# dbolya/yolact

Measured on AMD Instinct MI355X. Metric: images/sec (550x550, batch 8 per GPU), YOLACT yolact_resnet50 forward + Detect (Fast NMS), higher is better.
Workload: dtype f32 (fp32 in / fp32 accumulate / fp32 out; 93 % of the GEMM time on fp16x2 tiles = every fp32 operand as two fp16 pieces by round to nearest (22 significant bits + 2 signs: exact for ~2/3 of all fp32 values, one fp32 ulp otherwise), 3 exact piece products per product on the fp16 matrix pipe; measure

## Files before the change

### yolact_amd/csrc/common.h

```cpp
#pragma once
#include <hip/hip_runtime.h>
#include <stdint.h>

#define YMI_OK 0
#define YMI_EARG (-1)
#define YMI_ESHAPE (-2)
#define YMI_ENULL (-3)

typedef float f32x4 __attribute__((ext_vector_type(4)));
typedef float f32x16 __attribute__((ext_vector_type(16)));

static inline int ymi_launch_status() {
  hipError_t e = hipGetLastError();
  return e == hipSuccess ? YMI_OK : (int)e;
}

__device__ __forceinline__ int ymi_lane() { return threadIdx.x & 63; }

__device__ __forceinline__ int ymi_xcd_remap(int bid, int nwg) {
  const int q = nwg >> 3, r = nwg & 7, xcd = bid & 7, local = bid >> 3;
  const int base = (xcd < r) ? xcd * (q + 1) : r * (q + 1) + (xcd - r) * q;
  return base + local;
}

__host__ __device__ __forceinline__ void ymi_h2_scale(float amax, float &s, float &inv) {
  const unsigned u = __builtin_bit_cast(unsigned, amax);
  const int eb = (int)((u >> 23) & 0xff);
  int es = 267 - eb;
  if (eb == 0 || eb == 255) es = 127;
  es = es < 2 ? 2 : (es > 252 ? 252 : es);
  s = __builtin_bit_cast(float, (unsigned)es << 23);
  inv = __builtin_bit_cast(float, (unsigned)(254 - es) << 23);
}

#define YMI_AMAX_SUB 16
#define YMI_AMAX_STRIDE 64
struct ymi_amax_pre { float *sub; unsigned cur; };
__device__ __forceinline__ unsigned ymi_wave_umax63(unsigned v) {
  auto step = [](unsigned x, unsigned y) { return x > y ? x : y; };
  v = step(v, (unsigned)__builtin_amdgcn_update_dpp(0, (int)v, 0xb1, 0xf, 0xf, false));
  v = step(v, (unsigned)__builtin_amdgcn_update_dpp(0, (int)v, 0x4e, 0xf, 0xf, false));
  v = step(v, (unsigned)__builtin_amdgcn_update_dpp(0, (int)v, 0x114, 0xf, 0xf, false));
  v = step(v, (unsigned)__builtin_amdgcn_update_dpp(0, (int)v, 0x118, 0xf, 0xf, false));
  v = step(v, (unsigned)__builtin_amdgcn_update_dpp(0, (int)v, 0x142, 0xa, 0xf, false));
  v = step(v, (unsigned)__builtin_amdgcn_update_dpp(0, (int)v, 0x143, 0xc, 0xf, false));
  return v;
}
__device__ __forceinline__ ymi_amax_pre ymi_amax_prefetch(float *slot) {
  ymi_amax_pre p;
  const unsigned xcc = (unsigned)__builtin_amdgcn_s_getreg((3 << 11) | (0 << 6) | 20) & 7u;
  p.sub = slot ? slot + (2 * xcc + ((blockIdx.x + blockIdx.y) & 1)) * YMI_AMAX_STRIDE : nullptr;
  p.cur = 0xffffffffu;
  if (slot && (threadIdx.x & 63) == 63)
    p.cur = __hip_atomic_load(reinterpret_cast<const unsigned *>(p.sub), __ATOMIC_RELAXED, __HIP_MEMORY_SCOPE_WORKGROUP);
  return p;
}
// ... 27 lines not shown
```

### yolact_amd/csrc/conv_igemm.hip

```cpp
#include "common.h"
#include <stdlib.h>
#include <mutex>
#include <type_traits>
#include "../../include/yolact_amd.h"

namespace {

constexpr int BK = 32;
constexpr unsigned OOB = 0x80000000u;

typedef __attribute__((address_space(3))) void *lds_ptr_t;
typedef unsigned u32x4 __attribute__((ext_vector_type(4)));
typedef __bf16 bf16x8 __attribute__((ext_vector_type(8)));

struct Split3 { bf16x8 h, m, l; };

__device__ __forceinline__ Split3 split8(const f32x4 x0, const f32x4 x1) {
  const float x[8] = {x0[0], x0[1], x0[2], x0[3], x1[0], x1[1], x1[2], x1[3]};
  unsigned r1[8], r2[8];
#pragma unroll
  for (int e = 0; e < 8; ++e) {
    const float h = __builtin_bit_cast(float, __builtin_bit_cast(unsigned, x[e]) & 0xFFFF0000u);
    const float r = x[e] - h;
    r1[e] = __builtin_bit_cast(unsigned, r);
// ... 2 lines not shown
  }
  u32x4 ph, pm, pl;
#pragma unroll
  for (int q = 0; q < 4; ++q) {
    ph[q] = __builtin_amdgcn_perm(__builtin_bit_cast(unsigned, x[2 * q + 1]), __builtin_bit_cast(unsigned, x[2 * q]), 0x07060302u);
    pm[q] = __builtin_amdgcn_perm(r1[2 * q + 1], r1[2 * q], 0x07060302u);
    pl[q] = __builtin_amdgcn_perm(r2[2 * q + 1], r2[2 * q], 0x07060302u);
  }
  Split3 s;
  s.h = __builtin_bit_cast(bf16x8, ph); s.m = __builtin_bit_cast(bf16x8, pm); s.l = __builtin_bit_cast(bf16x8, pl);
  return s;
}


typedef _Float16 f16x8 __attribute__((ext_vector_type(8)));
struct Split2 { f16x8 h, l; };

__device__ __forceinline__ Split2 split8h(const f32x4 x0, const f32x4 x1, const float s) {
  const float x[8] = {x0[0], x0[1], x0[2], x0[3], x1[0], x1[1], x1[2], x1[3]};
  Split2 o;
#pragma unroll
  for (int e = 0; e < 8; ++e) {
    const float t = x[e] * s;
    const _Float16 h = (_Float16)t;
    o.h[e] = h;
    o.l[e] = (_Float16)(t - (float)h);
  }
  return o;
}

struct KParams {
  ymi_conv_desc d;
  int M, HoWo, tiles_n, nk;
  unsigned x_bytes, w_bytes;
  const float *offmask;
  int ldo, mask_is_prob, om_layout;
  long x_gs, w_gs, y_gs;
  const void *w3;
  unsigned w3_plane;
  unsigned w3_gs;
  const void *a2;
  unsigned a2_plane;
  long a2_gs;
  unsigned sc_gs;
  unsigned long long *trace;
  int abl;
};

__device__ __forceinline__ float act_apply(float v, int act) {
  switch (act) {
    case YMI_ACT_RELU: return v > 0.f ? v : 0.f;
    case YMI_ACT_LEAKY01: return v > 0.f ? v : 0.1f * v;
    case YMI_ACT_TANH: return tanhf(v);
    case YMI_ACT_SIGMOID: return 1.f / (1.f + expf(-v));
    default: return v;
  }
}

__device__ __forceinline__ void bilin_coord(int dst, float scale, int in_size, int &i0, int &i1, float &l1) {
  float src = scale * ((float)dst + 0.5f) - 0.5f;
  src = src < 0.f ? 0.f : src;
  i0 = (int)src;
  if (i0 > in_size - 1) i0 = in_size - 1;
  i1 = i0 + ((i0 < in_size - 1) ? 1 : 0);
  l1 = src - (float)i0;
}
// ... 118 lines not shown
  constexpr int NWAVE = WM * WN * WK, NTHR = 64 * NWAVE;
  constexpr int RPP = NTHR / 8;
  constexpr int NPL = (PREC == 2) ? 3 : 2;
  constexpr bool BPL = PREC >= 2;
  constexpr bool APL = PREC == 4;
  constexpr bool H2 = PREC >= 3;
  constexpr int RA = APL ? (2 * BM) / (16 * NWAVE) : BM / RPP, RB = BPL ? (NPL * BN) / (16 * NWAVE) : BN / RPP;
  static_assert((APL ? (2 * BM) % (16 * NWAVE) == 0 : BM % RPP == 0) && (BPL ? (NPL * BN) % (16 * NWAVE) == 0 : BN % RPP == 0),
                "tile rows must be a multiple of the rows per staging pass");
  static_assert(!APL || LOADER == 3, "pre-split A planes: pointwise loader only");
  constexpr int SUB = conv_sub_floats<BM, BN, PREC>();
  constexpr int STAGE = SUB * WK;
  constexpr int NS = (LOADER == 2) ? 2 : NSTAGE;
  constexpr int DMA_PER_STEP = (RA + RB) * WK;
  constexpr int ELD = BN + 4;
  constexpr int LDS_FLOATS = (NS * STAGE > WK * BM * ELD) ? NS * STAGE : WK * BM * ELD;
  static_assert(DMA_PER_STEP * (NS - 2) <= 63, "vmcnt is a 6-bit counter");
  static_assert(WM * WN * WK == 4 || WM * WN * WK == 8, "4 or 8 waves per block");
  static_assert(LOADER != 2 || WK == 1, "DCN gather runs without the K split");
  static_assert(PREC == 0 || PREC == 3 || LOADER != 2, "the DCN gather: exact-fp32 or fp16x2 (A split on the fly from the fp32 LDS image)");
  static_assert(!BPL || BN % 16 == 0, "16-bit planes: 16-row DMA pieces");
  __shared__ __attribute__((aligned(16))) float lds[LDS_FLOATS];

  const ymi_conv_desc &d = p.d;
  const int t = threadIdx.x;
  const int lane = t & 63, wave = __builtin_amdgcn_readfirstlane(t >> 6);
  const int wk = wave % WK, wmn = wave / WK;
  const int wm = wmn / WN, wn = wmn % WN;
  const int kq = t & 7, r0 = t >> 3;
  const int sl = kq ^ ((r0 >> 1) & 7);

  unsigned long long tr_t0 = 0, tr_loop = 0, tr_epi = 0, tr_tp = 0, tr_c = 0;
  if (p.trace) tr_t0 = __builtin_readcyclecounter();
  const int logical = ymi_xcd_remap(blockIdx.x, gridDim.x);
  const int tile_n = logical % p.tiles_n, tile_m = logical / p.tiles_n;
  const int m0 = tile_m * BM, n0 = tile_n * BN;

  const int grp = blockIdx.y;
  const __amdgpu_buffer_rsrc_t xrs = APL
      ? __builtin_amdgcn_make_buffer_rsrc((void *)((const char *)p.a2 + (size_t)grp * p.a2_gs), 0, (int)(2 * p.a2_plane), 0x00020000)
      : __builtin_amdgcn_make_buffer_rsrc((void *)(d.x + (size_t)grp * p.x_gs), 0, (int)p.x_bytes, 0x00020000);
  const __amdgpu_buffer_rsrc_t wrs = BPL
      ? __builtin_amdgcn_make_buffer_rsrc((void *)((const char *)p.w3 + (size_t)grp * p.w3_gs), 0, (int)(NPL * p.w3_plane), 0x00020000)
      : __builtin_amdgcn_make_buffer_rsrc((void *)(d.w + (size_t)grp * p.w_gs), 0, (int)p.w_bytes, 0x00020000);
  float sA = 1.f, invA = 1.f;
  if (H2) {
    float xam = d.x_amax ? ymi_amax_read(d.x_amax) : 0.f;
    if (d.x_amax_mul != 0.f) xam *= d.x_amax_mul;
    ymi_h2_scale(xam, sA, invA);
  }
  const ymi_amax_pre apre = ymi_amax_prefetch(d.y_amax);

  constexpr int C4 = BN / 4;
  constexpr int RSTEP = NTHR / C4;
  constexpr int RPT = BM / RSTEP;
  constexpr bool RES_PREFETCH = RPT <= 8;
  const int c4 = t % C4, rbase = t / C4;
  const int n = n0 + 4 * c4;
  const bool vec_res = (d.res_ld & 3) == 0 && ((((uintptr_t)d.res) & 15) == 0) && (n + 3 < d.Cout);
  f32x4 rpre[RES_PREFETCH ? RPT : 1];
  if (RES_PREFETCH && d.res_mode == YMI_RES_ADD && vec_res) {
#pragma unroll
    for (int i = 0; i < RPT; ++i) {
      const int m = m0 + rbase + RSTEP * i;
      const f32x4 z = {0.f, 0.f, 0.f, 0.f};
      rpre[i] = (m < p.M) ? *reinterpret_cast<const f32x4 *>(d.res + (size_t)m * d.res_ld + n) : z;
    }
  }

  const float *scp = H2 ? d.scale_h2 + (size_t)grp * p.sc_gs : d.scale;
  f32x4 sc = {1.f, 1.f, 1.f, 1.f}, bi = {0.f, 0.f, 0.f, 0.f};
// ... 594 lines not shown
      epilogue_general<BM, BN, WK, RPT, RSTEP, RES_PREFETCH>(p, es, sc, bi, rpre, m0, n, c4, rbase, vec_res, invA, apre);
    }
  }
  if (p.trace && t == 0) {
    const unsigned hw = __builtin_amdgcn_s_getreg((31 << 11) | (0 << 6) | 4);
    const unsigned xcc = __builtin_amdgcn_s_getreg((3 << 11) | (0 << 6) | 20);
    unsigned long long *o = p.trace + (size_t)blockIdx.x * 8;
    o[0] = ((unsigned long long)xcc << 32) | hw;
    o[1] = tr_t0; o[2] = tr_loop; o[3] = tr_epi; o[4] = __builtin_readcyclecounter(); o[5] = tr_tp; o[6] = tr_c;
  }
#endif
}

struct ProfRec { hipEvent_t e0, e1; double flops; int tile; int kind; };
constexpr int PROF_MAX = 4096;
ProfRec g_prof[PROF_MAX];
unsigned long long *g_trace = nullptr;
long g_trace_cap = 0;
int g_prof_n = 0, g_prof_alloc = 0, g_prof_on = 0;
std::mutex g_prof_mu;

constexpr int LDS_PER_CU = 160 * 1024, NUM_CU = 256;

template <int WM, int WN, int WK, int TM, int TN, int NS, bool ALL_LOADERS, int PREC>
int launch_cfg(const KParams &kp, int loader, hipStream_t s, int groups) {
  constexpr int BM = WM * TM * 32, BN = WN * TN * 32;
  constexpr int ns_eff_bytes = NS * conv_sub_floats<BM, BN, PREC>() * WK * 4, epi_bytes = WK * BM * (BN + 4) * 4;
  constexpr int static_lds = ns_eff_bytes > epi_bytes ? ns_eff_bytes : epi_bytes;
  KParams p = kp;
  const int tiles_m = (p.M + BM - 1) / BM;
  p.tiles_n = (p.d.Cout + BN - 1) / BN;
  const int grid = tiles_m * p.tiles_n;
  if (p.trace && (grid > g_trace_cap || groups > 1)) p.trace = nullptr;
  int dyn = 0;
  {
    int occ = LDS_PER_CU / static_lds;
    if (PREC >= 1) {
      constexpr int occ_regs = conv_occupancy<WM, WN, WK, TM, TN, NS, 0, PREC>();
      occ = occ < occ_regs ? occ : occ_regs;
    }
    const int k = (grid * groups + NUM_CU - 1) / NUM_CU;
    if (k < occ && !(p.abl & 8)) {
      const int want = LDS_PER_CU / (k + 1) + 1024;
      if (want > static_lds && want <= LDS_PER_CU / k) dyn = want - static_lds;
    }
  }
  const bool pointwise = p.d.kh == 1 && p.d.kw == 1 && p.d.pad == 0;
  if constexpr (PREC == 4) {
    if (loader != 0 || !pointwise) return YMI_EARG;
    hipLaunchKernelGGL((conv_igemm_f32<WM, WN, WK, TM, TN, NS, 3, 4>), dim3(grid, groups), dim3(64 * WM * WN * WK), dyn, s, p);
    return ymi_launch_status();
  } else
  if (loader == 0 && (groups > 1 || pointwise)) {
    hipLaunchKernelGGL((conv_igemm_f32<WM, WN, WK, TM, TN, NS, 3, PREC>), dim3(grid, groups), dim3(64 * WM * WN * WK), dyn, s, p);
  } else if (loader == 0) {
    hipLaunchKernelGGL((conv_igemm_f32<WM, WN, WK, TM, TN, NS, 0, PREC>), dim3(grid, groups), dim3(64 * WM * WN * WK), dyn, s, p);
  } else if constexpr (ALL_LOADERS) {
    if (loader == 1) hipLaunchKernelGGL((conv_igemm_f32<WM, WN, WK, TM, TN, NS, 1, PREC>), dim3(grid, groups), dim3(64 * WM * WN * WK), dyn, s, p);
    else if constexpr (PREC == 0) hipLaunchKernelGGL((conv_igemm_f32<WM, WN, WK, TM, TN, NS, 2, 0>), dim3(grid, groups), dim3(64 * WM * WN * WK), dyn, s, p);
    else if constexpr (PREC == 3) hipLaunchKernelGGL((conv_igemm_f32<WM, WN, WK, TM, TN, NS, 2, 3>), dim3(grid, groups), dim3(64 * WM * WN * WK), dyn, s, p);
    else return YMI_EARG;
  } else {
    return YMI_EARG;
  }
  return ymi_launch_status();
}
// ... 402 lines not shown
```

### yolact_amd/csrc/dcn.hip

```cpp
#include "common.h"
#include <stdlib.h>
#include <type_traits>
#include "../../include/yolact_amd.h"

int ymi_internal_prof_begin(double flops, int tile, int kind, hipStream_t s);
void ymi_internal_prof_end(int idx, hipStream_t s);

#ifndef YMI_A_AUX
#define YMI_A_AUX 0
#endif

namespace {

constexpr int BK = 32;
constexpr unsigned OOB = 0x80000000u;

typedef __attribute__((address_space(3))) void *lds_ptr_t;
typedef unsigned u32x4 __attribute__((ext_vector_type(4)));
typedef unsigned u32x3 __attribute__((ext_vector_type(3)));
typedef _Float16 f16x8 __attribute__((ext_vector_type(8)));
typedef _Float16 f16x4 __attribute__((ext_vector_type(4)));
struct Split2 { f16x8 h, l; };

struct DcnParams {
  const float *x, *offmask, *scale_h2, *bias, *x_amax;
  const void *w_h2;
  float *y, *y_amax;
  int B, H, W, Cin, ldx, Ho, Wo, Cout, stride, Kpad, ldo, ldy, act, mask_is_prob;
  int taps, kw, pad;
  const float *res; int res_ld, res_after_act;
  int M, HoWo, tiles_n, nk;
  int nk_split;
  long y_gs;
  unsigned x_bytes, om_bytes, w_plane;
  int om_layout;
  int abl;
  unsigned long long *trace;
  int trace_mode;
};

template <int WM, int WN, int TM, int TN, int RING>
constexpr int dcn_lds_floats() {
  constexpr int BM = WM * TM * 32, BN = WN * TN * 32;
  constexpr int pipe = 2 * (2 * BM * 16) + (RING + 2) * (2 * BN * 16), epi = BM * (BN + 4);
  return pipe > epi ? pipe : epi;
}
template <int WM, int WN, int TM, int TN, int RING, bool PLAIN>
constexpr int dcn_occupancy() {
  constexpr int occ = (160 * 1024) / (dcn_lds_floats<WM, WN, TM, TN, RING>() * 4);
  constexpr int nw = WM * WN, ra = (WM * TM * 32) / (8 * nw);
  constexpr int cap = (!PLAIN && (nw > 8 || (nw == 8 && ra > 1))) ? 1 : (WN * TN == 1 && nw <= 4) ? 4 : 2;
  return occ > cap ? cap : (occ < 1 ? 1 : occ);
}

template <int WM, int WN, int TM, int TN, int RING, bool PLAIN>
__global__ __launch_bounds__(64 * WM * WN, (dcn_occupancy<WM, WN, TM, TN, RING, PLAIN>() * (WM * WN) + 3) / 4)
void pipe_h2_k(const DcnParams p) {
#if defined(__HIP_DEVICE_COMPILE__)
  constexpr int BM = WM * TM * 32, BN = WN * TN * 32, NW = WM * WN, NT = 64 * NW;
  constexpr int RPP = NT / 8, RA = BM / RPP;
  constexpr int BUNITS = (2 * BN) / 16;
  constexpr int RB = (BUNITS + NW - 1) / NW;
  static_assert(BM % RPP == 0 && RA >= 1, "tile rows vs gather passes");
  static_assert(RING == 1 || RING == 2, "ring depth");
  constexpr int NSB = RING + 2;
  constexpr int A_STAGE = 2 * BM * 16, B_STAGE = 2 * BN * 16;
  constexpr int NC = PLAIN ? 1 : 4;
  constexpr int NG = NC * RA, NB = RB;
  constexpr int N_STEADY = RING * (NG + NB);
  static_assert(N_STEADY <= 63, "vmcnt is a 6-bit counter");
  constexpr int ELD = BN + 4;
  constexpr int LDS_FLOATS = dcn_lds_floats<WM, WN, TM, TN, RING>();
  __shared__ __attribute__((aligned(16))) float lds[LDS_FLOATS];
  float *const Abase = lds, *const Bbase = lds + 2 * A_STAGE;

  const int t = threadIdx.x;
  const int lane = t & 63, wave = __builtin_amdgcn_readfirstlane(t >> 6);
  const int wm = wave / WN, wn = wave % WN;
  const int kq = t & 7, r0 = t >> 3;
#ifdef YMI_DIAGNOSTICS
  unsigned long long tr_[10] = {0, 0, 0, 0, 0, 0, 0, 0, 0, 0}, tr_rt0 = 0;
  const bool tracing = p.trace != nullptr;
#define YMI_STAMP(i) do { if (tracing) tr_[i] = __builtin_amdgcn_s_memtime(); } while (0)
  if (tracing) tr_rt0 = __builtin_amdgcn_s_memrealtime();
  YMI_STAMP(0);
#else
#define YMI_STAMP(i) do { } while (0)
#endif

  const int logical = ymi_xcd_remap(blockIdx.x, gridDim.x);
  const int tile_n = logical % p.tiles_n, tile_m = logical / p.tiles_n;
  const int m0 = tile_m * BM, n0 = tile_n * BN;

  const __amdgpu_buffer_rsrc_t xrs = __builtin_amdgcn_make_buffer_rsrc((void *)p.x, 0, (int)p.x_bytes, 0x00020000);
  const __amdgpu_buffer_rsrc_t ors = __builtin_amdgcn_make_buffer_rsrc((void *)p.offmask, 0, (int)p.om_bytes, 0x00020000);
  const __amdgpu_buffer_rsrc_t wrs = __builtin_amdgcn_make_buffer_rsrc((void *)p.w_h2, 0, (int)(2 * p.w_plane), 0x00020000);

  float sA, invA;
  ymi_h2_scale(ymi_amax_read(p.x_amax), sA, invA);
  const ymi_amax_pre apre = ymi_amax_prefetch(p.y_amax);
#ifdef YMI_DIAGNOSTICS
  if (tracing && p.trace_mode == 2) {
    unsigned long long tt;
    asm volatile("s_memtime %0\n\ts_waitcnt lgkmcnt(0)" : "=s"(tt) : "s"(__builtin_amdgcn_readfirstlane(__builtin_bit_cast(int, sA))) : "memory");
    tr_[1] = tt;
  }
#endif

  constexpr int C4 = BN / 4, RSTEP = NT / C4, RPT = BM / RSTEP;
  const int c4 = t % C4, rbase = t / C4;
  const int n = n0 + 4 * c4;
  int g_iy0[RA], g_ix0[RA], g_ib[RA];
  unsigned g_om[RA];
  int a_st[RA];
#pragma unroll
  for (int i = 0; i < RA; ++i) {
    const int row = r0 + RPP * i, m = m0 + row;
    a_st[i] = row * 64 + (((kq >> 1) ^ ((row >> 2) & 3)) * 16) + (kq & 1) * 8;
    if (m < p.M) {
      const int b = m / p.HoWo, pix = m - b * p.HoWo;
      const int oy = pix / p.Wo, ox = pix - oy * p.Wo;
      g_iy0[i] = oy * p.stride - (PLAIN ? p.pad : 1);
      g_ix0[i] = ox * p.stride - (PLAIN ? p.pad : 1);
      g_ib[i] = b * p.H * p.W;
// ... 345 lines not shown
      o[10] = tr_rt0;
      o[11] = __builtin_amdgcn_s_memrealtime();
      o[12] = (unsigned long long)__builtin_amdgcn_s_getreg((31 << 11) | (0 << 6) | 4);
      o[13] = (unsigned long long)(__builtin_amdgcn_s_getreg((3 << 11) | (0 << 6) | 20) & 7u);
      o[14] = (unsigned long long)my_nk;
      o[15] = 1;
    }
  }
#endif
#undef YMI_STAMP
#endif
}

template <int WM, int WN, int TM, int TN, int RING, bool PLAIN>
int launch_dcn_k(DcnParams p, hipStream_t s) {
  constexpr int BM = WM * TM * 32, BN = WN * TN * 32;
  p.tiles_n = (p.Cout + BN - 1) / BN;
  const int grid = ((p.M + BM - 1) / BM) * p.tiles_n;
  int dyn = 0;
  {
    constexpr int LDS_PER_CU = 160 * 1024, static_lds = dcn_lds_floats<WM, WN, TM, TN, RING>() * 4;
    const int occ = dcn_occupancy<WM, WN, TM, TN, RING, PLAIN>(), k = (grid * ((p.nk + p.nk_split - 1) / p.nk_split) + 255) / 256;
#ifdef YMI_DIAGNOSTICS
    const bool cap_on = !(p.abl & 64);
#else
    const bool cap_on = true;
#endif
    if (k < occ && cap_on) {
      const int want = LDS_PER_CU / (k + 1) + 1024;
      if (want > static_lds && want <= LDS_PER_CU / k) dyn = want - static_lds;
    }
  }
  const int splits = (p.nk + p.nk_split - 1) / p.nk_split;
  hipLaunchKernelGGL((pipe_h2_k<WM, WN, TM, TN, RING, PLAIN>), dim3(grid, splits), dim3(64 * WM * WN), dyn, s, p);
  return ymi_launch_status();
}

template <int WM, int WN, int TM, int TN, int RING = 2>
int launch_dcn(const DcnParams &p, bool plain, hipStream_t s) {
  return plain ? launch_dcn_k<WM, WN, TM, TN, RING, true>(p, s) : launch_dcn_k<WM, WN, TM, TN, RING, false>(p, s);
}

}

int ymi_internal_splitk_fixup(const float *part, long gstride, int S, long M, int Cout, int ldy, float *y, const float *scale,
                              const float *bias, const float *res, int res_ld, int act, int res_after_act, float *y_amax,
                              hipStream_t s);

namespace {

int run_pipe(const ymi_conv_desc *d, const float *offmask, int ldo, int mask_is_prob, int om_layout, int base_tile, int prof_kind,
             hipStream_t s) {
  const bool plain = offmask == nullptr;
  const ymi_conv_seg &g0 = d->seg[0];
  const long HoWo = (long)d->Ho * d->Wo, M = (long)d->B * HoWo;
  if (plain) {
    if (!((d->kh == 3 && d->kw == 3 && d->pad == 1) || (d->kh == 1 && d->kw == 1 && d->pad == 0))) return YMI_EARG;
  } else if (d->kh != 3 || d->kw != 3 || d->pad != 1) return YMI_EARG;
  if (d->Cin % 32 != 0 || d->Kpad != d->kh * d->kw * d->Cin) return YMI_EARG;
  if (d->nseg != 1 || g0.n0 != 0 || g0.n1 < d->Cout || (d->Cout & 3) || (g0.row_stride & 3) || (((uintptr_t)g0.ptr) & 15) ||
      g0.batch_stride != HoWo * g0.row_stride || g0.act > YMI_ACT_LEAKY01 || g0.act < 0)
    return YMI_EARG;
  if (d->res_mode != YMI_RES_NONE && (!plain || d->res_mode != YMI_RES_ADD || (d->res_ld & 3) || (((uintptr_t)d->res) & 15))) return YMI_EARG;
  if (!d->w_h2 || !d->scale_h2 || !d->x_amax || (((uintptr_t)d->w_h2) & 15)) return YMI_ENULL;
  if (M * (long)(plain ? 1 : ldo) >= (1L << 29) || M * (long)g0.row_stride >= (1L << 31)) return YMI_ESHAPE;
  const int S = d->split_k > 1 ? d->split_k : 1;
// ... 73 lines not shown
```

### yolact_amd/csrc/wgemm.hip

```cpp
#include "common.h"
#include <stdlib.h>
#include <type_traits>
#include "../../include/yolact_amd.h"

int ymi_internal_prof_begin(double flops, int tile, int kind, hipStream_t s);
void ymi_internal_prof_end(int idx, hipStream_t s);

namespace {

typedef __attribute__((address_space(3))) void *lds_ptr_t;
typedef _Float16 f16x8 __attribute__((ext_vector_type(8)));
typedef unsigned u32x4 __attribute__((ext_vector_type(4)));
constexpr unsigned OOB = 0x80000000u;

constexpr int BM = 128, BN = 256;
constexpr int A_BYTES = 2 * BM * 64, B_BYTES = 2 * BN * 64, STAGE = A_BYTES + B_BYTES, NST = 3;
constexpr int OFF_SC = NST * STAGE, WG_LDS = OFF_SC + 2 * BN * 4;
constexpr int NPC = 12;

struct WgParams {
  const char *v, *u;
  const float *uinv, *x_amax;
  float *m;
  long v_gs, u_gs, m_gs;
  unsigned v_plane, u_plane;
  int G, T, C, Ng, cout_pad, tiles_m, tiles_n, nitems;
  float amax_mul;
  unsigned long long *trace;
  int abl;
};

__global__ __launch_bounds__(512, 2) void wgemm_k(const WgParams p) {
#if defined(__HIP_DEVICE_COMPILE__)
  __shared__ __attribute__((aligned(16))) char lds[WG_LDS];
  const int t = threadIdx.x, lane = t & 63, wave = __builtin_amdgcn_readfirstlane(t >> 6);
  const bool producer = wave >= 4;
  const int lr = lane & 31, hh = lane >> 5;
  const int nk = p.C >> 5;
  const int nb = (int)gridDim.x, b0 = (int)blockIdx.x;
  const int my_items = (p.nitems - b0 + nb - 1) / nb;
  const int nsteps = my_items * nk;
#ifdef YMI_DIAGNOSTICS
  unsigned long long tr_[8] = {0, 0, 0, 0, 0, 0, 0, 0};
  const bool tracing = p.trace != nullptr;
  tr_[0] = __builtin_amdgcn_s_memtime();
#endif
#define WG_WAIT_VM(N) asm volatile("s_waitcnt vmcnt(%0)" ::"n"(N) : "memory")
#define WG_BARRIER() asm volatile("s_waitcnt lgkmcnt(0)\n\ts_barrier" ::: "memory")
  auto decode = [&](int it, int &g, int &tm, int &tn) {
    tn = it % p.tiles_n;
    const int r = it / p.tiles_n;
    tm = r % p.tiles_m;
    g = r / p.tiles_m;
  };

  if (producer) {
    const int pw = wave - 4;
    int a_row[4], a_dst[4], b_row[8], b_dst[8];
    unsigned a_ko[4], b_ko[8];
#pragma unroll
    for (int i = 0; i < 4; ++i) {
      const int q = pw + 4 * i, plane = q >> 3, rg = q & 7;
      const int row = rg * 16 + (lane >> 2), lsl = (lane & 3) ^ ((row >> 2) & 3);
      a_row[i] = row; a_ko[i] = (unsigned)plane * p.v_plane + 16u * lsl; a_dst[i] = plane * (BM * 64) + rg * 1024;
    }
#pragma unroll
    for (int i = 0; i < 8; ++i) {
      const int q = pw + 4 * i, plane = q >> 4, rg = q & 15;
      const int row = rg * 16 + (lane >> 2), lsl = (lane & 3) ^ ((row >> 2) & 3);
      b_row[i] = row; b_ko[i] = (unsigned)plane * p.u_plane + 16u * lsl; b_dst[i] = A_BYTES + plane * (BN * 64) + rg * 1024;
    }
    int ridx = 0, rkc = 0;
    __amdgpu_buffer_rsrc_t vrs, urs, srs;
    unsigned a_vo[4], b_vo[8];
    int sc_par = 0;
    auto open_item = [&](int idx) {
      const bool live = idx < my_items;
      int g = 0, tm = 0, tn = 0;
      decode(live ? b0 + idx * nb : 0, g, tm, tn);
      vrs = __builtin_amdgcn_make_buffer_rsrc((void *)(p.v + (size_t)g * p.v_gs), 0, live ? (int)p.v_gs : 0, 0x00020000);
      urs = __builtin_amdgcn_make_buffer_rsrc((void *)(p.u + (size_t)g * p.u_gs), 0, live ? (int)p.u_gs : 0, 0x00020000);
      srs = __builtin_amdgcn_make_buffer_rsrc((void *)(p.uinv + (size_t)g * p.cout_pad), 0, live ? p.cout_pad * 4 : 0, 0x00020000);
#pragma unroll
      for (int i = 0; i < 4; ++i) {
        const int row = tm * BM + a_row[i];
        a_vo[i] = (live && row < p.T && !(p.abl & 2)) ? a_ko[i] + (unsigned)(row * p.C) * 2u : OOB;
      }
#pragma unroll
      for (int i = 0; i < 8; ++i) {
        const int row = tn * BN + b_row[i];
        b_vo[i] = (live && row < p.cout_pad && !(p.abl & 4)) ? b_ko[i] + (unsigned)(row * p.C) * 2u : OOB;
      }
      const int n = tn * BN + 4 * lane;
      __builtin_amdgcn_raw_ptr_buffer_load_lds(srs, (lds_ptr_t)(lds + OFF_SC + sc_par * (BN * 4)), 16, (live && n < p.cout_pad) ? (unsigned)n * 4u : OOB, 0, 0, 0);
      sc_par ^= 1;
    };
    auto request = [&](int stage) {
      if (rkc == 0) open_item(ridx);
      char *dst = lds + stage * STAGE;
      const unsigned so = (unsigned)rkc * 64u;
#pragma unroll
      for (int i = 0; i < 4; ++i) __builtin_amdgcn_raw_ptr_buffer_load_lds(vrs, (lds_ptr_t)(dst + a_dst[i]), 16, a_vo[i], so, 0, 0);
#pragma unroll
      for (int i = 0; i < 8; ++i) __builtin_amdgcn_raw_ptr_buffer_load_lds(urs, (lds_ptr_t)(dst + b_dst[i]), 16, b_vo[i], so, 0, 0);
      if (++rkc == nk) { rkc = 0; ++ridx; }
    };
    request(0);
    request(1);
    WG_WAIT_VM(NPC);
#ifdef YMI_DIAGNOSTICS
    tr_[1] = __builtin_amdgcn_s_memtime();
#endif
// ... 40 lines not shown
#pragma unroll
      for (int s2 = 0; s2 < 2; ++s2) {
        const char *ub = sb + (s2 ? uo1 : uo0), *vb = sb + (s2 ? vo1 : vo0);
        f16x8 vh[2], vl[2];
#pragma unroll
        for (int j = 0; j < 2; ++j) {
          vh[j] = *reinterpret_cast<const f16x8 *>(vb + j * 2048);
          vl[j] = *reinterpret_cast<const f16x8 *>(vb + BM * 64 + j * 2048);
        }
#pragma unroll
        for (int ip = 0; ip < 2; ++ip) {
          f16x8 uh[2], ul[2];
#pragma unroll
          for (int ii = 0; ii < 2; ++ii) {
            uh[ii] = *reinterpret_cast<const f16x8 *>(ub + (2 * ip + ii) * 2048);
            ul[ii] = *reinterpret_cast<const f16x8 *>(ub + BN * 64 + (2 * ip + ii) * 2048);
          }
#pragma unroll
          for (int pr = 0; pr < 3; ++pr)
#pragma unroll
            for (int ii = 0; ii < 2; ++ii)
#pragma unroll
              for (int j = 0; j < 2; ++j)
#ifdef YMI_DIAGNOSTICS
                if (!(p.abl & 8))
#endif
                acc[2 * ip + ii][j] = __builtin_amdgcn_mfma_f32_32x32x16_f16(pr == 0 ? ul[ii] : uh[ii], pr == 1 ? vl[j] : vh[j], acc[2 * ip + ii][j], 0, 0, 0);
        }
      }
      st = st == 2 ? 0 : st + 1;
      if (++kc == nk) {
        kc = 0;
        int g, tm, tn;
        decode(b0 + idx * nb, g, tm, tn);
        ++idx;
        const float *sc = reinterpret_cast<const float *>(lds + OFF_SC + sc_par * (BN * 4));
        sc_par ^= 1;
        float *mg = p.m + (size_t)g * p.m_gs;
#pragma unroll
        for (int j = 0; j < 2; ++j) {
          const int row = tm * BM + 32 * (2 * wp + j) + lr;
          const bool rok = row < p.T;
#pragma unroll
          for (int i = 0; i < 4; ++i)
#pragma unroll
            for (int gq = 0; gq < 4; ++gq) {
              const int nl = 32 * (4 * wc + i) + 8 * gq + 4 * hh, n = tn * BN + nl;
              const f32x4 s4 = *reinterpret_cast<const f32x4 *>(sc + nl);
              f32x4 v;
#pragma unroll
              for (int e = 0; e < 4; ++e) { v[e] = acc[i][j][4 * gq + e] * (s4[e] * invA); acc[i][j][4 * gq + e] = 0.f; }
#ifdef YMI_DIAGNOSTICS
              if (p.abl & 1) continue;
              if (p.abl & 16) { if (rok && n < p.Ng) __builtin_nontemporal_store(v, reinterpret_cast<f32x4 *>(mg + (size_t)row * p.Ng + n)); continue; }
#endif
              if (rok && n < p.Ng) *reinterpret_cast<f32x4 *>(mg + (size_t)row * p.Ng + n) = v;
            }
        }
      }
#ifdef YMI_DIAGNOSTICS
      const unsigned long long a_ = tracing ? __builtin_amdgcn_s_memtime() : 0ull;
#endif
      WG_BARRIER();
#ifdef YMI_DIAGNOSTICS
      if (tracing) tr_[3] += __builtin_amdgcn_s_memtime() - a_;
#endif
    }
// ... 11 lines not shown
      for (int i = 0; i < 8; ++i) o_[i] = tr_[i];
      o_[14] = (unsigned long long)nsteps;
      o_[15] = 1;
    }
  }
#endif
#endif
}

}

int ymi_internal_wgemm(const void *v, const void *u, const float *uinv, const float *x_amax, float amax_mul, float *m, int G, long T,
                       int C, int Ng, int cout_pad, double prof_flops, int prof_kind, hipStream_t s) {
  if (!v || !u || !uinv || !x_amax || !m) return YMI_ENULL;
  if (C % 32 != 0 || C < 64 || (Ng & 3) || G <= 0 || T <= 0) return YMI_ESHAPE;
  if (T * (long)C * 4 >= (1L << 31) || (long)cout_pad * C * 4 >= (1L << 31) || T * (long)Ng >= (1L << 29)) return YMI_ESHAPE;
  if ((((uintptr_t)v) | ((uintptr_t)u) | ((uintptr_t)m) | ((uintptr_t)uinv)) & 15) return YMI_ESHAPE;
  WgParams p;
  p.v = (const char *)v; p.u = (const char *)u; p.uinv = uinv; p.x_amax = x_amax; p.m = m;
  p.v_plane = (unsigned)(T * C * 2); p.v_gs = 2L * T * C * 2;
  p.u_plane = (unsigned)((long)cout_pad * C * 2); p.u_gs = 2L * cout_pad * C * 2;
  p.m_gs = T * (long)Ng;
  p.G = G; p.T = (int)T; p.C = C; p.Ng = Ng; p.cout_pad = cout_pad;
  p.tiles_m = (int)((T + BM - 1) / BM); p.tiles_n = (Ng + BN - 1) / BN; p.nitems = G * p.tiles_m * p.tiles_n;
  p.amax_mul = amax_mul;
  p.trace = nullptr; p.abl = 0;
#ifdef YMI_DIAGNOSTICS
  { const char *e = getenv("YMI_WGEMM_ABLATE"); p.abl = e ? atoi(e) : 0; }
  { const char *e = getenv("YMI_WGEMM_TRACE"); p.trace = e ? (unsigned long long *)strtoull(e, nullptr, 0) : nullptr; }
#endif
  int dev = 0, cus = 256;
  hipGetDevice(&dev);
  hipDeviceGetAttribute(&cus, hipDeviceAttributeMultiprocessorCount, dev);
  const int pr = ymi_internal_prof_begin(prof_flops, YMI_TILE_H2 | YMI_TILE_WG_128x256, prof_kind, s);
  hipLaunchKernelGGL(wgemm_k, dim3((unsigned)(p.nitems < cus ? p.nitems : cus)), dim3(512), 0, s, p);
  const int rc = ymi_launch_status();
  ymi_internal_prof_end(pr, s);
  return rc;
}
```

### yolact_amd/csrc/detect.hip

```cpp
#include "common.h"
#include <stdlib.h>
#include "../../include/yolact_amd.h"

namespace {

typedef int i32x4 __attribute__((ext_vector_type(4)));

constexpr int NT = 1024;
constexpr int NT_MAX = 1024;
constexpr int SORT_N = 256;

#define YMI_STAMP(i) do { if (trace && threadIdx.x == 0) trace[(size_t)tblk * 16 + (i)] = __builtin_readcyclecounter(); } while (0)

__device__ __forceinline__ unsigned f2key(float f) {
  unsigned u = __float_as_uint(f);
  return (u & 0x80000000u) ? ~u : (u | 0x80000000u);
}

__device__ __forceinline__ f32x4 decode_box(const float *loc, const float *pr) {
  const float cx = pr[0] + (loc[0] * 0.1f) * pr[2];
  const float cy = pr[1] + (loc[1] * 0.1f) * pr[3];
  const float w = pr[2] * expf(loc[2] * 0.2f);
  const float h = pr[3] * expf(loc[3] * 0.2f);
  f32x4 b;
// ... 36 lines not shown
    sum += __shfl_xor(sum, 1);
    sum += __shfl_xor(sum, 2);
    if (live) for (int c = sub; c < C; c += 4) row[c] = row[c] / sum;
  }
  float best = -__builtin_inff();
  int bi = 0x7fffffff;
  if (live) for (int c = 1 + sub; c < C; c += 4) { const float v = row[c]; if (v > best) { best = v; bi = c - 1; } }
#pragma unroll
  for (int off = 1; off <= 2; off <<= 1) {
    const float ob = __shfl_xor(best, off);
    const int oi = __shfl_xor(bi, off);
    if (ob > best || (ob == best && oi < bi)) { best = ob; bi = oi; }
  }
  if (live && sub == 0) {
    const int kp = best > thresh ? 1 : 0;
    keep[(size_t)b * P + p0 + j] = kp;
    kflag[j] = (unsigned char)kp;
    maxsc[(size_t)b * P + p0 + j] = best;
    argmax[(size_t)b * P + p0 + j] = bi;
    if (kp) atomicAdd(&blk_cnt, 1);
  }
  __syncthreads();
  if (t == 0 && blk_cnt) atomicAdd(&num_keep[b], blk_cnt);
  const int nfg = C - 1;
  for (int i = t; i < nfg * 64; i += 256) {
    const int c = i >> 6, jj = i & 63;
    if (jj < np) {
      const float v = s[jj * C + c + 1];
      scores_t[((size_t)b * nfg + c) * P + p0 + jj] = kflag[jj] ? v : __uint_as_float(__float_as_uint(v) | 0x80000000u);
    }
  }
}

struct SelShared {
  unsigned hist[2 * (NT_MAX / 64)];
  unsigned long long comp[SORT_N];
  unsigned cnt_gt;
  unsigned wave_tot[2][NT_MAX / 64];
};

__device__ __forceinline__ unsigned wave_sum_to_lane63(unsigned v) {
  v += (unsigned)__builtin_amdgcn_update_dpp(0, (int)v, 0xb1, 0xf, 0xf, false);
  v += (unsigned)__builtin_amdgcn_update_dpp(0, (int)v, 0x4e, 0xf, 0xf, false);
  v += (unsigned)__builtin_amdgcn_update_dpp(0, (int)v, 0x114, 0xf, 0xf, false);
  v += (unsigned)__builtin_amdgcn_update_dpp(0, (int)v, 0x118, 0xf, 0xf, false);
  v += (unsigned)__builtin_amdgcn_update_dpp(0, (int)v, 0x142, 0xa, 0xf, false);
  v += (unsigned)__builtin_amdgcn_update_dpp(0, (int)v, 0x143, 0xc, 0xf, false);
  return v;
}

__device__ __forceinline__ unsigned wave_incl_scan(unsigned v, int lane) {
#pragma unroll
  for (int off = 1; off < 64; off <<= 1) {
    const unsigned o = (unsigned)__shfl_up((int)v, off);
    if (lane >= off) v += o;
  }
  return v;
}

template <int NTH>
__device__ __forceinline__ unsigned block_excl_scan(unsigned v, SelShared &sh, int slot, unsigned &total) {
  constexpr int NW = NTH / 64;
  const int t = threadIdx.x, lane = t & 63, w = t >> 6;
  const unsigned inc = wave_incl_scan(v, lane);
  if (lane == 63) sh.wave_tot[slot][w] = inc;
  __syncthreads();
  unsigned before = 0, tot = 0;
#pragma unroll
  for (int ww = 0; ww < NW; ++ww) { const unsigned x = sh.wave_tot[slot][ww]; if (ww < w) before += x; tot += x; }
  total = tot;
  return before + inc - v;
// ... 34 lines not shown
               OP " %[m6], %[k6], %[cd]\n\t" OP " %[m7], %[k7], %[cd]\n\t"                                          \
               "s_bcnt1_i32_b64 %[n0], %[m0]\n\ts_bcnt1_i32_b64 %[n1], %[m1]\n\ts_bcnt1_i32_b64 %[n2], %[m2]\n\t"   \
               "s_bcnt1_i32_b64 %[n3], %[m3]\n\ts_bcnt1_i32_b64 %[n4], %[m4]\n\ts_bcnt1_i32_b64 %[n5], %[m5]\n\t"   \
               "s_bcnt1_i32_b64 %[n6], %[m6]\n\ts_bcnt1_i32_b64 %[n7], %[m7]\n\t"                                  \
               "s_add_u32 %[n0], %[n0], %[n1]\n\ts_add_u32 %[n2], %[n2], %[n3]\n\ts_add_u32 %[n4], %[n4], %[n5]\n\t" \
               "s_add_u32 %[n6], %[n6], %[n7]\n\ts_add_u32 %[n0], %[n0], %[n2]\n\ts_add_u32 %[n4], %[n4], %[n6]\n\t" \
               "s_add_u32 %[n0], %[n0], %[n4]\n\ts_add_u32 %[c], %[c], %[n0]"                                        \
               : [c] "+s"(c), [m0] "=&s"(m0), [m1] "=&s"(m1), [m2] "=&s"(m2), [m3] "=&s"(m3), [m4] "=&s"(m4),         \
                 [m5] "=&s"(m5), [m6] "=&s"(m6), [m7] "=&s"(m7), [n0] "=&s"(n0), [n1] "=&s"(n1), [n2] "=&s"(n2),      \
                 [n3] "=&s"(n3), [n4] "=&s"(n4), [n5] "=&s"(n5), [n6] "=&s"(n6), [n7] "=&s"(n7)                       \
               : [k0] "v"(k[0]), [k1] "v"(k[1]), [k2] "v"(k[2]), [k3] "v"(k[3]), [k4] "v"(k[4]), [k5] "v"(k[5]),      \
                 [k6] "v"(k[6]), [k7] "v"(k[7]), [cd] "s"(cand)                                                       \
               : "scc")
template <int EPT, bool STRICT>
__device__ __forceinline__ unsigned wave_count_keys(const unsigned (&keys)[EPT > 0 ? EPT : 1], unsigned cand_any) {
  static_assert(EPT % 8 == 0, "keys per thread: a multiple of 8");
  const unsigned cand = (unsigned)__builtin_amdgcn_readfirstlane((int)cand_any);
  unsigned c = 0;
#pragma unroll
  for (int g = 0; g < EPT / 8; ++g) {
    const unsigned *k = &keys[8 * g];
    unsigned long long m0, m1, m2, m3, m4, m5, m6, m7;
    unsigned n0, n1, n2, n3, n4, n5, n6, n7;
    if (STRICT) YMI_CMP8("v_cmp_gt_u32_e64");
    else YMI_CMP8("v_cmp_ge_u32_e64");
  }
  return c;
}
#undef YMI_CMP8

template <int NTH>
__device__ __forceinline__ int reg_index(int t, int j) { return 4 * (t + NTH * (j >> 2)) + (j & 3); }

template <int EPT, int NTH, typename KeyFn>
__device__ __forceinline__ void block_topk_regs(const unsigned (&keys)[EPT > 0 ? EPT : 1], KeyFn key, int n, int k, SelShared &sh,
                                unsigned long long *trace = nullptr, long tblk = 0) {
  constexpr int NW = NTH / 64;
  const int t = threadIdx.x, lane = t & 63, w = t >> 6;
  const int rounds = EPT > 0 ? EPT : (n + NTH - 1) / NTH;
  auto key_at = [&](int j) -> unsigned {
    const int i = t + NTH * j;
    return i < n ? key(i) : 0u;
  };
  auto index_of = [&](int j) -> int { return EPT > 0 ? reg_index<NTH>(t, j) : t + NTH * j; };
  auto block_count = [&](unsigned cand, bool strict, int slot) -> unsigned {
    unsigned c = 0;
    if (EPT > 0) {
      c = strict ? wave_count_keys<EPT, true>(keys, cand) : wave_count_keys<EPT, false>(keys, cand);
      if (lane == 0) sh.hist[slot * NW + w] = c;
    } else {
      for (int j = 0; j < rounds; ++j) {
        const unsigned kk = key_at(j);
        c += (strict ? kk > cand : kk >= cand) ? 1u : 0u;
      }
      c = wave_sum_to_lane63(c);
      if (lane == 63) sh.hist[slot * NW + w] = c;
    }
    __syncthreads();
    unsigned tot = 0;
#pragma unroll
    for (int ww = 0; ww < NW; ++ww) tot += sh.hist[slot * NW + ww];
    return tot;
  };
  unsigned T = 0;
  for (int bit = 31; bit >= 0; --bit) {
    const unsigned cand = T | (1u << bit);
    if (block_count(cand, false, bit & 1) >= (unsigned)k) T = cand;
  }
  __syncthreads();
  YMI_STAMP(2);
  const unsigned n_gt = block_count(T, true, 0);
  const unsigned n_ge = block_count(T, false, 1);
  const unsigned krem = (unsigned)k - n_gt;
  if (t < SORT_N) sh.comp[t] = 0ull;
  if (t == 0) sh.cnt_gt = 0;
  const bool all_eq = n_ge - n_gt == krem;
  auto wins = [&](unsigned kj) -> bool { return kj != 0 && (all_eq ? kj >= T : kj > T); };
  unsigned mine = 0;
  if constexpr (EPT > 0) {
#pragma unroll
    for (int j = 0; j < EPT; ++j) mine += wins(keys[j]) ? 1u : 0u;
  } else {
    for (int j = 0; j < rounds; ++j) mine += wins(key_at(j)) ? 1u : 0u;
  }
  unsigned total;
  unsigned pos = block_excl_scan<NTH>(mine, sh, 0, total);
  if (mine) {
    if constexpr (EPT > 0) {
#pragma unroll
      for (int j = 0; j < EPT; ++j)
        if (wins(keys[j])) {
          sh.comp[pos] = ((unsigned long long)keys[j] << 32) | (unsigned)(0xffffffffu - (unsigned)index_of(j));
          ++pos;
        }
    } else {
      for (int j = 0; j < rounds; ++j) {
        const unsigned kj = key_at(j);
        if (wins(kj)) {
          sh.comp[pos] = ((unsigned long long)kj << 32) | (unsigned)(0xffffffffu - (unsigned)index_of(j));
          ++pos;
        }
      }
    }
  }
  if (!all_eq) {
    unsigned base_eq = 0;
    if constexpr (EPT > 0) {
#pragma unroll
      for (int g = 0; g < EPT / 4; ++g) {
// ... 315 lines not shown
```

Measured before the change: 2266.

## Place GEMM tiles per XCD with column groups to cut cross-die traffic

Adds an XCD placement helper that maps each block to a contiguous range of logical tiles per XCD. The conv and DCN kernels can now split the output columns into 2, 4 or 8 groups, so each XCD reads only a slice of the weights. The group count comes from a simple host-side model that compares activation bytes against weight bytes. The wgemm persistent kernel now walks items in per-XCD contiguous ranges and rounds its grid to a multiple of 8. The aim is better L2 locality and less fabric traffic, at the cost of more index arithmetic and possible load imbalance.

```diff
diff --git a/yolact_amd/csrc/common.h b/yolact_amd/csrc/common.h
--- a/yolact_amd/csrc/common.h
+++ b/yolact_amd/csrc/common.h
@@ -17,11 +17,9 @@
 
 __device__ __forceinline__ int ymi_lane() { return threadIdx.x & 63; }
 
-__device__ __forceinline__ int ymi_xcd_remap(int bid, int nwg) {
-  const int q = nwg >> 3, r = nwg & 7, xcd = bid & 7, local = bid >> 3;
-  const int base = (xcd < r) ? xcd * (q + 1) : r * (q + 1) + (xcd - r) * q;
-  return base + local;
-}
+#include "xcd_place.h"
+
+__device__ __forceinline__ int ymi_xcd_remap(int bid, int nwg) { return ymi_xcd_place(bid, nwg); }
 
 __host__ __device__ __forceinline__ void ymi_h2_scale(float amax, float &s, float &inv) {
   const unsigned u = __builtin_bit_cast(unsigned, amax);
diff --git a/yolact_amd/csrc/conv_igemm.hip b/yolact_amd/csrc/conv_igemm.hip
--- a/yolact_amd/csrc/conv_igemm.hip
+++ b/yolact_amd/csrc/conv_igemm.hip
@@ -58,6 +58,7 @@
 struct KParams {
   ymi_conv_desc d;
   int M, HoWo, tiles_n, nk;
+  int xgroups;
   unsigned x_bytes, w_bytes;
   const float *offmask;
   int ldo, mask_is_prob, om_layout;
@@ -242,11 +243,13 @@
 
   unsigned long long tr_t0 = 0, tr_loop = 0, tr_epi = 0, tr_tp = 0, tr_c = 0;
   if (p.trace) tr_t0 = __builtin_readcyclecounter();
-  const int logical = ymi_xcd_remap(blockIdx.x, gridDim.x);
-  const int tile_n = logical % p.tiles_n, tile_m = logical / p.tiles_n;
+  const int per_grp = (int)gridDim.x;
+  const int glog = ymi_xcd_place((int)(blockIdx.x + gridDim.x * blockIdx.y), per_grp * (int)gridDim.y);
+  const int grp = glog / per_grp;
+  int tile_m, tile_n;
+  ymi_colgroup_tile(glog - grp * per_grp, per_grp / p.tiles_n, p.tiles_n, p.xgroups, tile_m, tile_n);
   const int m0 = tile_m * BM, n0 = tile_n * BN;
 
-  const int grp = blockIdx.y;
   const __amdgpu_buffer_rsrc_t xrs = APL
       ? __builtin_amdgcn_make_buffer_rsrc((void *)((const char *)p.a2 + (size_t)grp * p.a2_gs), 0, (int)(2 * p.a2_plane), 0x00020000)
       : __builtin_amdgcn_make_buffer_rsrc((void *)(d.x + (size_t)grp * p.x_gs), 0, (int)p.x_bytes, 0x00020000);
@@ -907,6 +910,13 @@
   p.tiles_n = (p.d.Cout + BN - 1) / BN;
   const int grid = tiles_m * p.tiles_n;
   if (p.trace && (grid > g_trace_cap || groups > 1)) p.trace = nullptr;
+  p.xgroups = 1;
+  if (groups == 1) {
+    const ymi_conv_desc &d = p.d;
+    const double in_px = (d.kh == 1 && d.kw == 1) ? (double)p.M : (double)d.B * d.H * d.W;
+    const double w_bytes = (double)d.Cout * d.Kpad * (PREC == 2 || PREC == 1 ? 6.0 : 4.0);
+    p.xgroups = ymi_xcd_pick_groups(in_px * d.Cin * 4.0, w_bytes, tiles_m, p.tiles_n);
+  }
   int dyn = 0;
   {
     int occ = LDS_PER_CU / static_lds;
diff --git a/yolact_amd/csrc/dcn.hip b/yolact_amd/csrc/dcn.hip
--- a/yolact_amd/csrc/dcn.hip
+++ b/yolact_amd/csrc/dcn.hip
@@ -30,6 +30,7 @@
   int taps, kw, pad;
   const float *res; int res_ld, res_after_act;
   int M, HoWo, tiles_n, nk;
+  int xgroups;
   int nk_split;
   long y_gs;
   unsigned x_bytes, om_bytes, w_plane;
@@ -88,8 +89,8 @@
 #define YMI_STAMP(i) do { } while (0)
 #endif
 
-  const int logical = ymi_xcd_remap(blockIdx.x, gridDim.x);
-  const int tile_n = logical % p.tiles_n, tile_m = logical / p.tiles_n;
+  int tile_m, tile_n;
+  ymi_colgroup_tile(ymi_xcd_remap(blockIdx.x, gridDim.x), (int)gridDim.x / p.tiles_n, p.tiles_n, p.xgroups, tile_m, tile_n);
   const int m0 = tile_m * BM, n0 = tile_n * BN;
 
   const __amdgpu_buffer_rsrc_t xrs = __builtin_amdgcn_make_buffer_rsrc((void *)p.x, 0, (int)p.x_bytes, 0x00020000);
@@ -501,6 +502,12 @@
     }
   }
   const int splits = (p.nk + p.nk_split - 1) / p.nk_split;
+  p.xgroups = 1;
+  if (splits == 1 || grid % 8 == 0) {
+    const double in_px = p.taps == 1 ? (double)p.M : (double)p.B * p.H * p.W;
+    const double a_bytes = in_px * p.Cin * 4.0 + (double)p.om_bytes, w_bytes = 2.0 * p.w_plane;
+    p.xgroups = ymi_xcd_pick_groups(a_bytes, w_bytes, grid / p.tiles_n, p.tiles_n);
+  }
   hipLaunchKernelGGL((pipe_h2_k<WM, WN, TM, TN, RING, PLAIN>), dim3(grid, splits), dim3(64 * WM * WN), dyn, s, p);
   return ymi_launch_status();
 }
diff --git a/yolact_amd/csrc/wgemm.hip b/yolact_amd/csrc/wgemm.hip
--- a/yolact_amd/csrc/wgemm.hip
+++ b/yolact_amd/csrc/wgemm.hip
@@ -37,9 +37,11 @@
   const bool producer = wave >= 4;
   const int lr = lane & 31, hh = lane >> 5;
   const int nk = p.C >> 5;
-  const int nb = (int)gridDim.x, b0 = (int)blockIdx.x;
-  const int my_items = (p.nitems - b0 + nb - 1) / nb;
+  const int nbx = (int)gridDim.x >> 3, xr = (int)blockIdx.x & 7, j0 = (int)blockIdx.x >> 3;
+  const int r_base = ymi_xcd_base(xr, p.nitems), r_cnt = ymi_xcd_count(xr, p.nitems);
+  const int my_items = j0 < r_cnt ? (r_cnt - j0 + nbx - 1) / nbx : 0;
   const int nsteps = my_items * nk;
+  auto item_of = [&](int idx) { return r_base + j0 + idx * nbx; };
 #ifdef YMI_DIAGNOSTICS
   unsigned long long tr_[8] = {0, 0, 0, 0, 0, 0, 0, 0};
   const bool tracing = p.trace != nullptr;
@@ -77,7 +79,7 @@
     auto open_item = [&](int idx) {
       const bool live = idx < my_items;
       int g = 0, tm = 0, tn = 0;
-      decode(live ? b0 + idx * nb : 0, g, tm, tn);
+      decode(live ? item_of(idx) : 0, g, tm, tn);
       vrs = __builtin_amdgcn_make_buffer_rsrc((void *)(p.v + (size_t)g * p.v_gs), 0, live ? (int)p.v_gs : 0, 0x00020000);
       urs = __builtin_amdgcn_make_buffer_rsrc((void *)(p.u + (size_t)g * p.u_gs), 0, live ? (int)p.u_gs : 0, 0x00020000);
       srs = __builtin_amdgcn_make_buffer_rsrc((void *)(p.uinv + (size_t)g * p.cout_pad), 0, live ? p.cout_pad * 4 : 0, 0x00020000);
@@ -184,7 +186,7 @@
       if (++kc == nk) {
         kc = 0;
         int g, tm, tn;
-        decode(b0 + idx * nb, g, tm, tn);
+        decode(item_of(idx), g, tm, tn);
         ++idx;
         const float *sc = reinterpret_cast<const float *>(lds + OFF_SC + sc_par * (BN * 4));
         sc_par ^= 1;
@@ -262,8 +264,9 @@
   int dev = 0, cus = 256;
   hipGetDevice(&dev);
   hipDeviceGetAttribute(&cus, hipDeviceAttributeMultiprocessorCount, dev);
+  const int cap = (cus & ~7) > 8 ? (cus & ~7) : 8, want = (p.nitems + 7) & ~7;
   const int pr = ymi_internal_prof_begin(prof_flops, YMI_TILE_H2 | YMI_TILE_WG_128x256, prof_kind, s);
-  hipLaunchKernelGGL(wgemm_k, dim3((unsigned)(p.nitems < cus ? p.nitems : cus)), dim3(512), 0, s, p);
+  hipLaunchKernelGGL(wgemm_k, dim3((unsigned)(want < cap ? want : cap)), dim3(512), 0, s, p);
   const int rc = ymi_launch_status();
   ymi_internal_prof_end(pr, s);
   return rc;
diff --git a/yolact_amd/csrc/xcd_place.h b/yolact_amd/csrc/xcd_place.h
--- /dev/null
+++ b/yolact_amd/csrc/xcd_place.h
@@ -0,0 +1,37 @@
+#pragma once
+
+#if defined(__HIPCC__) || defined(__HIP__)
+#define YMI_HD __host__ __device__ __forceinline__
+#else
+#define YMI_HD inline
+#endif
+
+YMI_HD int ymi_xcd_base(int x, int n) {
+  const int q = n >> 3, r = n & 7;
+  return x < r ? x * (q + 1) : r * (q + 1) + (x - r) * q;
+}
+YMI_HD int ymi_xcd_count(int x, int n) { return (n >> 3) + (x < (n & 7) ? 1 : 0); }
+
+YMI_HD int ymi_xcd_place(int lin, int n) { return ymi_xcd_base(lin & 7, n) + (lin >> 3); }
+
+YMI_HD void ymi_colgroup_tile(int logical, int tiles_m, int tiles_n, int a, int &tm, int &tn) {
+  const int per = tiles_n / a, grp = logical / (tiles_m * per), r = logical - grp * (tiles_m * per);
+  tm = r / per;
+  tn = grp * per + (r - (r / per) * per);
+}
+
+YMI_HD double ymi_xcd_fabric_bytes(double a_bytes, double w_bytes, int a) { return a_bytes * a + w_bytes * 8.0 / a; }
+
+YMI_HD int ymi_xcd_pick_groups(double a_bytes, double w_bytes, int tiles_m, int tiles_n) {
+  int best = 1;
+  if (tiles_m < 8) return best;
+  double cost = ymi_xcd_fabric_bytes(a_bytes, w_bytes, 1) * 0.9;
+  for (int a = 2; a <= 8; a *= 2) {
+    if (tiles_n % a != 0) continue;
+    const double c = ymi_xcd_fabric_bytes(a_bytes, w_bytes, a);
+    if (c < cost) { cost = c; best = a; }
+  }
+  return best;
+}
+
+#undef YMI_HD
```

Result: no change. 2271 (median of 6 runs) (+0.2%).

## Replace bitwise top-k threshold search with 12-bit radix histogram selection

Applied to the files above, without the earlier changes.

For the register-resident key path, the 32-iteration bit-by-bit threshold search (one block-wide count and barrier per bit) is replaced by a radix select. It first finds the common prefix of all nonzero keys via block AND/OR reductions, then narrows the threshold 12 bits at a time using shared-memory atomic histograms and a block scan. This cuts the number of block-wide synchronisation rounds. In exchange it adds LDS atomics and a 32 KB histogram to shared memory, which may reduce occupancy.

```diff
diff --git a/yolact_amd/csrc/detect.hip b/yolact_amd/csrc/detect.hip
--- a/yolact_amd/csrc/detect.hip
+++ b/yolact_amd/csrc/detect.hip
@@ -92,11 +92,16 @@
   }
 }
 
+constexpr int RADIX_BITS = 12;
+constexpr int RADIX_BINS = 1 << RADIX_BITS;
 struct SelShared {
   unsigned hist[2 * (NT_MAX / 64)];
   unsigned long long comp[SORT_N];
   unsigned cnt_gt;
   unsigned wave_tot[2][NT_MAX / 64];
+  unsigned rhist[2][RADIX_BINS] __attribute__((aligned(16)));
+  unsigned red[3][NT_MAX / 64];
+  unsigned sel[3];
 };
 
 __device__ __forceinline__ unsigned wave_sum_to_lane63(unsigned v) {
@@ -197,6 +202,66 @@
 template <int NTH>
 __device__ __forceinline__ int reg_index(int t, int j) { return 4 * (t + NTH * (j >> 2)) + (j & 3); }
 
+template <int EPT, int NTH>
+__device__ __forceinline__ void radix_threshold(const unsigned (&keys)[EPT], unsigned k, SelShared &sh, unsigned &T,
+                                                unsigned &n_gt, bool &all_eq) {
+  constexpr int NW = NTH / 64, BPT = RADIX_BINS / NTH;
+  static_assert(BPT == 4, "the boundary search reads four bins per thread");
+  const int t = threadIdx.x, lane = t & 63, w = t >> 6;
+  const uint4 z4 = {0u, 0u, 0u, 0u};
+  reinterpret_cast<uint4 *>(sh.rhist[0])[t] = z4;
+  reinterpret_cast<uint4 *>(sh.rhist[1])[t] = z4;
+  unsigned a = ~0u, o = 0u, nzl = 0u;
+#pragma unroll
+  for (int j = 0; j < EPT; ++j) if (keys[j]) { a &= keys[j]; o |= keys[j]; ++nzl; }
+#pragma unroll
+  for (int off = 32; off > 0; off >>= 1) { a &= (unsigned)__shfl_xor((int)a, off); o |= (unsigned)__shfl_xor((int)o, off); }
+  nzl = wave_sum_to_lane63(nzl);
+  if (lane == 63) { sh.red[0][w] = a; sh.red[1][w] = o; sh.red[2][w] = nzl; }
+  __syncthreads();
+  unsigned nz = 0;
+  a = ~0u; o = 0u;
+#pragma unroll
+  for (int ww = 0; ww < NW; ++ww) { a &= sh.red[0][ww]; o |= sh.red[1][ww]; nz += sh.red[2][ww]; }
+  if (nz < k) { T = 0u; n_gt = nz; all_eq = true; return; }
+  const unsigned diff = a ^ o;
+  int bits = diff ? 32 - __clz((int)diff) : 0;
+  unsigned pre = bits >= 32 ? 0u : a & (~0u << bits);
+  unsigned need = k, above = 0u, cnt = nz;
+  for (int p = 0; bits > 0; ++p) {
+    const int wd = bits < RADIX_BITS ? bits : RADIX_BITS, sft = bits - wd;
+    const unsigned hm = bits >= 32 ? 0u : ~0u << bits, dm = (1u << wd) - 1u;
+    unsigned *h = sh.rhist[p & 1];
+#pragma unroll
+    for (int j = 0; j < EPT; ++j) {
+      const unsigned kj = keys[j];
+      if (kj != 0u && (kj & hm) == pre) atomicAdd(&h[(kj >> sft) & dm], 1u);
+    }
+    __syncthreads();
+    const uint4 hv = reinterpret_cast<const uint4 *>(h)[t];
+    reinterpret_cast<uint4 *>(h)[t] = z4;
+    unsigned tot;
+    const unsigned before = block_excl_scan<NTH>(hv.x + hv.y + hv.z + hv.w, sh, p & 1, tot);
+    unsigned acc = tot - before - (hv.x + hv.y + hv.z + hv.w);
+    const unsigned hb[4] = {hv.x, hv.y, hv.z, hv.w};
+#pragma unroll
+    for (int b = 3; b >= 0; --b) {
+      if (acc < need && acc + hb[b] >= need) { sh.sel[0] = (unsigned)(4 * t + b); sh.sel[1] = acc; sh.sel[2] = hb[b]; }
+      acc += hb[b];
+    }
+    __syncthreads();
+    pre |= sh.sel[0] << sft;
+    above += sh.sel[1];
+    need -= sh.sel[1];
+    cnt = sh.sel[2];
+    bits = sft;
+    if (cnt == need) break;
+  }
+  T = pre;
+  n_gt = above;
+  all_eq = cnt == need;
+}
+
 template <int EPT, int NTH, typename KeyFn>
 __device__ __forceinline__ void block_topk_regs(const unsigned (&keys)[EPT > 0 ? EPT : 1], KeyFn key, int n, int k, SelShared &sh,
                                 unsigned long long *trace = nullptr, long tblk = 0) {
@@ -227,19 +292,25 @@
     for (int ww = 0; ww < NW; ++ww) tot += sh.hist[slot * NW + ww];
     return tot;
   };
-  unsigned T = 0;
-  for (int bit = 31; bit >= 0; --bit) {
-    const unsigned cand = T | (1u << bit);
-    if (block_count(cand, false, bit & 1) >= (unsigned)k) T = cand;
-  }
-  __syncthreads();
-  YMI_STAMP(2);
-  const unsigned n_gt = block_count(T, true, 0);
-  const unsigned n_ge = block_count(T, false, 1);
+  unsigned T = 0, n_gt;
+  bool all_eq;
+  if constexpr (EPT > 0) {
+    radix_threshold<EPT, NTH>(keys, (unsigned)k, sh, T, n_gt, all_eq);
+    YMI_STAMP(2);
+  } else {
+    for (int bit = 31; bit >= 0; --bit) {
+      const unsigned cand = T | (1u << bit);
+      if (block_count(cand, false, bit & 1) >= (unsigned)k) T = cand;
+    }
+    __syncthreads();
+    YMI_STAMP(2);
+    n_gt = block_count(T, true, 0);
+    const unsigned n_ge = block_count(T, false, 1);
+    all_eq = n_ge - n_gt == (unsigned)k - n_gt;
+  }
   const unsigned krem = (unsigned)k - n_gt;
   if (t < SORT_N) sh.comp[t] = 0ull;
   if (t == 0) sh.cnt_gt = 0;
-  const bool all_eq = n_ge - n_gt == krem;
   auto wins = [&](unsigned kj) -> bool { return kj != 0 && (all_eq ? kj >= T : kj > T); };
   unsigned mine = 0;
   if constexpr (EPT > 0) {
```

New measurement: 2279 before, 2311 after (median of 6 runs). 1.4% higher.
